# daigo0927/tf-raft

Hardware: AMD Instinct MI355X
Metric: image-pairs/sec at 448×512 iters_pred=24; final-iter EPE vs TF ref (higher is better)
Workload: dtype f32; 1 GPU; RAFT forward BASELINE configs[1]: batch 4/GPU 448x512 iters_pred=24 random weights; pairs_per_gpu=4, global_batch=4, parallelism=dp1, collective=none

## Files before the change

### tf_raft_amd/csrc/mask_upsample.hip

```cpp
#include "conv_mfma.h"

namespace {
struct MaskUpArgs {
    const float *a;
    int lda;
    const float *wp;
    const float *bias;
    const float *flow;
    float *out;
    int B, h, w;
    float scale;
};

constexpr int MU_TH = 4, MU_TW = 16, MU_LDA = 40, MU_ABUF = 64 * MU_LDA, MU_PXS = 592, MU_N = 576, MU_K = 256;

__global__ void __launch_bounds__(512) mask_upsample_kernel(MaskUpArgs p) {
    __shared__ __attribute__((aligned(16))) float sa[2 * MU_ABUF];
    __shared__ __attribute__((aligned(16))) float sm[32 * MU_PXS];
    __shared__ float2 sf[6 * 18];

    const int tid = threadIdx.x, lane = tid & 63;
    const int wv = __builtin_amdgcn_readfirstlane(tid >> 6);
    const int G = lane >> 4, LR = lane & 15;
    const int rbp = wv & 1, cg = wv >> 1;
    const int tiles_x = (p.w + MU_TW - 1) / MU_TW, tiles_y = (p.h + MU_TH - 1) / MU_TH;
    const int ntiles = p.B * tiles_x * tiles_y;
  for (int tile = blockIdx.x; tile < ntiles; tile += gridDim.x) {
    const int bid = raft_xcd_remap(tile, ntiles);
    const int tx = bid % tiles_x, ty = (bid / tiles_x) % tiles_y, b = bid / (tiles_x * tiles_y);
    const int y0 = ty * MU_TH, x0 = tx * MU_TW;
    const int M = p.B * p.h * p.w;

    const __amdgpu_buffer_rsrc_t rsa = __builtin_amdgcn_make_buffer_rsrc(
        (void *)p.a, 0, (int)((((long)M - 1) * p.lda + MU_K) * 4), 0x00020000);
    const __amdgpu_buffer_rsrc_t rsw = __builtin_amdgcn_make_buffer_rsrc((void *)p.wp, 0, MU_K * MU_N * 4, 0x00020000);

    const int spx = tid >> 3, sc4 = tid & 7;
    const int syy = y0 + (spx >> 4), sxx = x0 + (spx & 15);
    const bool sok = (syy < p.h) & (sxx < p.w);
    const unsigned soff = sok ? (unsigned)((((b * p.h + syy) * p.w + sxx) * p.lda + sc4 * 4) * 4) : RAFT_OOB;
    f32x4 ra;
    auto gload = [&](int c) { ra = __builtin_bit_cast(f32x4, __builtin_amdgcn_raw_buffer_load_b128(rsa, (int)soff, c * 128, 0)); };
    auto lstore = [&](int buf) { *(f32x4 *)(sa + buf * MU_ABUF + spx * MU_LDA + sc4 * 4) = ra; };
    const int a_lane = ((2 * rbp) * 16 + LR) * MU_LDA + G * 4;
    f32x4 fa[2][2], fb[2][9];
    auto frag_a = [&](int buf, int kk, f32x4 *f) {
#pragma unroll
        for (int i = 0; i < 2; ++i) f[i] = *(const f32x4 *)(sa + buf * MU_ABUF + a_lane + i * 16 * MU_LDA + kk * 16);
    };
    const unsigned b_lane = (unsigned)(((G * MU_N) + cg * 144 + LR) * 16);
    auto frag_b = [&](int c, int kk, f32x4 *f) {
        const unsigned row = (unsigned)((c * 8 + kk * 4) * MU_N) * 16u;
#pragma unroll
        for (int j = 0; j < 9; ++j)
            f[j] = __builtin_bit_cast(f32x4, __builtin_amdgcn_raw_buffer_load_b128(rsw, (int)(b_lane + j * 256), (int)row, 0));
    };
    f32x4 acc[2][9];
#pragma unroll
    for (int i = 0; i < 2; ++i)
#pragma unroll
        for (int j = 0; j < 9; ++j) acc[i][j] = f32x4{0.f, 0.f, 0.f, 0.f};

    constexpr int NCH = MU_K / 32;
    gload(0);
    frag_b(0, 0, fb[0]);
    if (tid < 108) {
        const int yy = y0 - 1 + tid / 18, xx = x0 - 1 + tid % 18;
        float2 f = make_float2(0.f, 0.f);
        if (yy >= 0 && yy < p.h && xx >= 0 && xx < p.w) {
            f = *(const float2 *)(p.flow + ((int64_t)(b * p.h + yy) * p.w + xx) * 2);
            f.x *= 8.f;
            f.y *= 8.f;
        }
        sf[tid] = f;
    }
    lstore(0);
    raft_barrier_lds();
    gload(1);
    frag_a(0, 0, fa[0]);
#pragma unroll
    for (int c = 0; c < NCH; ++c) {
        const int buf = c & 1;
#pragma unroll
        for (int kk = 0; kk < 2; ++kk) {
            const int cur = kk;
            if (kk == 0) {
                frag_a(buf, 1, fa[1]);
                frag_b(c, 1, fb[1]);
            } else if (c + 1 < NCH) {
                lstore(buf ^ 1);
                if (c + 2 < NCH) gload(c + 2);
                raft_barrier_lds();
                frag_a(buf ^ 1, 0, fa[0]);
                frag_b(c + 1, 0, fb[0]);
            }
#pragma unroll
            for (int r = 0; r < 4; ++r)
#pragma unroll
                for (int i = 0; i < 2; ++i)
#pragma unroll
                    for (int j = 0; j < 9; ++j)
                        acc[i][j] = __builtin_amdgcn_mfma_f32_16x16x4f32(fa[cur][i][r], fb[cur][j][r], acc[i][j], 0, 0, 0);
        }
    }

    float bias[9];
#pragma unroll
    for (int j = 0; j < 9; ++j) bias[j] = p.bias[cg * 144 + j * 16 + LR];
#pragma unroll
    for (int half = 0; half < 2; ++half) {
        raft_barrier_lds();
        if (rbp == half) {
#pragma unroll
            for (int i = 0; i < 2; ++i)
#pragma unroll
                for (int j = 0; j < 9; ++j)
#pragma unroll
                    for (int r = 0; r < 4; ++r)
                        sm[(i * 16 + 4 * G + r) * MU_PXS + cg * 144 + j * 16 + LR] = (acc[i][j][r] + bias[j]) * p.scale;
        }
        raft_barrier_lds();
#pragma unroll
        for (int t = 0; t < 4; ++t) {
            const int item = tid + 512 * t;
            const int px = item >> 6, sub = item & 63;
            const int row = 2 * half + (px >> 4), col = px & 15;
            const int y = y0 + row, x = x0 + col;
            if (y >= p.h || x >= p.w) continue;
            const float *tl = sm + px * MU_PXS + sub * 9;
            float v[9], mx = -INFINITY;
#pragma unroll
            for (int k = 0; k < 9; ++k) {
                v[k] = tl[k];
                mx = fmaxf(mx, v[k]);
            }
            float s = 0.f;
#pragma unroll
            for (int k = 0; k < 9; ++k) {
                v[k] = __builtin_amdgcn_exp2f((v[k] - mx) * 1.44269504088896341f);
                s += v[k];
            }
            const float inv = 1.0f / s;
            float ox = 0.f, oy = 0.f;
#pragma unroll
            for (int k = 0; k < 9; ++k) {
                const float2 nb = sf[(row + k / 3) * 18 + col + k % 3];
                const float wk = v[k] * inv;
                ox += wk * nb.x;
                oy += wk * nb.y;
            }
            float2 *o = (float2 *)p.out + ((int64_t)b * (8 * p.h) + (8 * y + (sub >> 3))) * (int64_t)(8 * p.w) + (8 * x + (sub & 7));
            *o = make_float2(ox, oy);
        }
// ... 20 lines not shown
```

### tf_raft_amd/csrc/conv_wino4.h

```cpp
#pragma once
#include "conv_mfma.h"

typedef float f32x2 __attribute__((ext_vector_type(2)));
typedef unsigned int u32x2 __attribute__((ext_vector_type(2)));

#include <type_traits>
#include <utility>

#ifdef RAFT_WINO4_SCALAR
struct alignas(8) w4v2 {
    float x, y;
    __device__ __forceinline__ float operator[](int i) const { return i ? y : x; }
};
__device__ __forceinline__ w4v2 operator+(w4v2 a, w4v2 b) { return {a.x + b.x, a.y + b.y}; }
__device__ __forceinline__ w4v2 operator-(w4v2 a, w4v2 b) { return {a.x - b.x, a.y - b.y}; }
__device__ __forceinline__ w4v2 operator*(float k, w4v2 a) { return {k * a.x, k * a.y}; }
#else
typedef f32x2 w4v2;
#endif

template <class F, int... I>
__device__ __forceinline__ void w4_static_for_impl(F &f, std::integer_sequence<int, I...>) {
    (f(std::integral_constant<int, I>{}), ...);
}
template <int N, class F>
__device__ __forceinline__ void w4_static_for(F &&f) {
    w4_static_for_impl(f, std::make_integer_sequence<int, N>{});
}
#define W4_TAPS(X)                                                                                                       \
    X(0) X(1) X(2) X(3) X(4) X(5) X(6) X(7) X(8) X(9) X(10) X(11) X(12) X(13) X(14) X(15) X(16) X(17) X(18) X(19) X(20) X(21)   \
    X(22) X(23) X(24) X(25) X(26) X(27) X(28) X(29) X(30) X(31) X(32) X(33) X(34) X(35)

#ifndef RAFT_WINO4_PF
#define RAFT_WINO4_PF 7
#endif
#ifdef RAFT_WINO4_NOSB
#define W4_SB()
#else
#define W4_SB() __builtin_amdgcn_sched_barrier(0)
#endif
#ifdef RAFT_WINO4_NOSNOP
#define W4_PAD ""
#else
#define W4_PAD "s_nop 1\n\t"
#endif
#define W4_MFMA4                                                                                                          \
    W4_PAD "v_mfma_f32_16x16x4_f32 %0, %2, %4, %0\n\tv_mfma_f32_16x16x4_f32 %1, %2, %6, %1\n\t"                          \
           "v_mfma_f32_16x16x4_f32 %0, %3, %5, %0\n\tv_mfma_f32_16x16x4_f32 %1, %3, %7, %1"
#ifndef RAFT_WINO4_ATAPS
#define RAFT_WINO4_ATAPS 31
#endif
#ifndef RAFT_WINO4_ABL
#define RAFT_WINO4_ABL 0
#endif

namespace wino4 {
constexpr float PA = 0.625f, PB = 1.5f;
constexpr float A2 = PA * PA, B2 = PB * PB, SS = A2 + B2, PP = A2 * B2, A3 = A2 * PA, B3 = B2 * PB;
constexpr int TW = 64, HWP = TW + 2;
constexpr int RS = 1124;
constexpr int NTHR = 256;
constexpr int PF = RAFT_WINO4_PF, NR = 8;
constexpr int W4_ATAPS = RAFT_WINO4_ATAPS;
#ifndef RAFT_WINO4_LAG
#define RAFT_WINO4_LAG 12
#endif
constexpr int LOAD_SLOT0 = 0, STORE_LAG = RAFT_WINO4_LAG;
static_assert(PF >= 1 && PF < NR, "prefetch distance must fit the fragment ring");
__device__ __forceinline__ constexpr int tap_row(int ph, int row) { return ph == 0 ? 1 + row : (ph == 1 ? 3 + row : 5 * row); }
}

#pragma clang diagnostic push
#pragma clang diagnostic ignored "-Wunused-lambda-capture"
template <int EPI, int KS = 1, int PRE = 0, int STATS = 0>
__global__ void __launch_bounds__(256, 1) conv_wino4_kernel(ConvArgs p) {
    using namespace wino4;
    static_assert(EPI == EPI_LINEAR || EPI == EPI_RELU || EPI == EPI_RES, "winograd F(4x4) kernel: linear / relu / residual epilogues");
    static_assert(KS == 1 || KS == 2, "K split: 1 or 2");
    static_assert((!PRE && !STATS) || KS == 1, "encoder variants: two row blocks per workgroup");
    constexpr int TH = KS == 1 ? 8 : 4, HH = TH + 2, HP = HH * HWP;
    constexpr int A_BUF = HH * RS + 16;
    constexpr int NA = (HP * 4 * KS + NTHR - 1) / NTHR;
    static_assert(LOAD_SLOT0 + NA - 1 + STORE_LAG < 60, "halo writes must precede the chunk's barrier (slot 60)");
    __shared__ __attribute__((aligned(16))) float smem[2 * KS * A_BUF];

    const int tid = threadIdx.x, lane = tid & 63;
    const int w = __builtin_amdgcn_readfirstlane(tid >> 6);
    const int G = lane >> 4, LR = lane & 15;
    const int rb = KS == 1 ? (w & 1) : 0, cbp = KS == 1 ? (w >> 1) : (w & 1), ks = KS == 1 ? 0 : (w >> 1);
    const int tiles_x = (p.W + TW - 1) / TW, tiles_y = (p.H + TH - 1) / TH;
    const int ntn = p.npad / 64;
    const int M = p.B * p.H * p.W;

    const int bid = raft_xcd_remap(blockIdx.x, gridDim.x);
    int mt = bid / ntn, nt = bid - mt * ntn;
#ifdef RAFT_WINO4_XCD
    {
        const int nwg = gridDim.x, xcd = blockIdx.x & 7, idx = blockIdx.x >> 3;
        if ((nwg & 7) == 0 && (ntn & 7) == 0) {
            const int per = ntn >> 3;
            nt = xcd + 8 * (idx % per);
            mt = idx / per;
        } else if ((nwg & 7) == 0 && 8 % ntn == 0) {
            const int g = 8 / ntn;
            nt = xcd % ntn;
            mt = idx * g + xcd / ntn;
        }
    }
#endif
    const int tx0 = mt % tiles_x, ty0 = (mt / tiles_x) % tiles_y, b = mt / (tiles_x * tiles_y);
    const int y0 = ty0 * TH, x0 = tx0 * TW;
    const int n0 = nt * 64;
    const int cin = p.c0 + p.c1;
    const int nch = cin >> 4;
    const int nst = nch / KS;

    const __amdgpu_buffer_rsrc_t rs0 = raft_stage_src0(p, M, p.c0), rsw = raft_stage_weights(p, 36, cin);
// ... 122 lines not shown
        }
        W[par][0][j] = (R[3][j] - SS * R[1][j]) + PP * e0;
        W[par][1][j] = (e5 - SS * R[2][j]) + PP * R[0][j];
    };
    w4v2 V[6];
    auto s2_calc = [&](const w4v2 *wr, int tx) {
        if (RAFT_WINO4_ABL & 16) {
            V[tx] = wr[tx];
            return;
        }
        if (tx == 0) {
            V[0] = (wr[4] - SS * wr[2]) + PP * wr[0];
        } else if (tx == 1) {
            const w4v2 t1 = wr[4] - B2 * wr[2], t2 = wr[3] - B2 * wr[1];
            V[1] = t1 + PA * t2;
            V[2] = t1 - PA * t2;
        } else if (tx == 3) {
            const w4v2 t1 = wr[4] - A2 * wr[2], t2 = wr[3] - A2 * wr[1];
            V[3] = t1 + PB * t2;
            V[4] = t1 - PB * t2;
        } else if (tx == 5) {
            V[5] = (wr[5] - SS * wr[3]) + PP * wr[1];
        }
    };

    next_source(0);
#pragma unroll
    for (int i = 0; i < NA; ++i) gload_item(i);
#pragma unroll
    for (int q = 0; q < PF; ++q) frag_b(q);
#pragma unroll
    for (int i = 0; i < NA; ++i) lstore_item(i, 0);
    raft_barrier_lds();
#pragma unroll
    for (int j = 0; j < 6; ++j) {
#pragma unroll
        for (int r = 0; r < 4; ++r) R[r][j] = (RAFT_WINO4_ABL & 2) ? w4v2{1.f, 1.f} : rd(0, r + 1, j, 0);
        s1_pair(0, 0, j);
    }
    s2_calc(W[0][0], 0);

    auto chunk = [&](auto buf_c, int c) {
        constexpr int BUF = decltype(buf_c)::value;
        next_source(c + 1);
        w4_static_for<6>([&](auto inst_c) {
            constexpr int inst = decltype(inst_c)::value;
            constexpr int h = inst / 3, ph = inst % 3, par = inst & 1;
            constexpr int n_h = ph == 2 ? 1 - h : h;
            constexpr int n_buf = (ph == 2 && h == 1) ? 1 - BUF : BUF;
            if (inst == 5) raft_barrier_lds();
            w4_static_for<12>([&](auto u_c) {
                constexpr int u = decltype(u_c)::value;
                constexpr int row = u / 6, tx = u % 6, j = u >> 1;
                constexpr int q = inst * 12 + u;
                constexpr int t = tap_row(ph, row) * 6 + tx;
                if (!(RAFT_WINO4_ABL & 1)) frag_b((q + PF) % 72, q + PF == 72);
                if (!(RAFT_WINO4_ABL & 2)) {
                    if constexpr (ph == 1 && (u & 1) == 0) {
                        e0 = rd(BUF, 0, j, h);
                        e5 = rd(BUF, 5, j, h);
                    }
                    if constexpr (ph == 2 && (u & 1) == 0) {
#pragma unroll
                        for (int r = 0; r < 4; ++r) R[r][j] = rd(n_buf, r + 1, j, n_h);
                    }
                }
                if constexpr ((u & 1) == 1) {
                    if constexpr (ph == 0) s1_pair(par ^ 1, 1, j);
                    if constexpr (ph == 1) s1_edge(par ^ 1, j);
                    if constexpr (ph == 2) s1_pair(par ^ 1, 0, j);
                }
                {
                    constexpr int li = q - LOAD_SLOT0, si = q - LOAD_SLOT0 - STORE_LAG;
                    if constexpr (li >= 0 && li < NA) gload_item(li);
                    if constexpr (si >= 0 && si < NA) lstore_item(si, 1 - BUF);
                }
                W4_SB();
                mma4(std::integral_constant<int, t>{}, V[tx][0], V[tx][1], fb[q & (NR - 1)]);
                W4_SB();
                if constexpr (u < 11) s2_calc(W[par][(u + 1) / 6], (u + 1) % 6);
                if constexpr (u == 11) s2_calc(W[par ^ 1][0], 0);
            });
        });
    };
    for (int st = 0; st < nst; st += 2) {
        chunk(std::integral_constant<int, 0>{}, st);
        chunk(std::integral_constant<int, 1>{}, st + 1);
    }

    asm volatile("s_nop 15\n\ts_nop 15" ::: "memory");
    __builtin_amdgcn_sched_barrier(0);

    constexpr bool HAS_E0 = EPI == EPI_RES;
    const EpiBuffers eb = raft_epi_buffers<EPI>(p, M);
    const bool interior = (y0 + TH <= p.H) & (x0 + TW <= p.W);
    int tid_e = threadIdx.x;
    asm volatile("" : "+v"(tid_e));
    const int G_e = (tid_e >> 4) & 3, LR_e = tid_e & 15, rb_e = (tid_e >> 6) & 1, cbp_e = tid_e >> 7;
    const int xb = x0 + 16 * G_e;
    const int ks_e = KS == 1 ? 0 : (tid_e >> 7), cb_e = KS == 1 ? cbp_e : ((tid_e >> 6) & 1), w_e = tid_e >> 6;
    constexpr int NROW = KS == 1 ? 4 : 2;
    unsigned bo[NROW], be[NROW];
    bool rowok[NROW];
#pragma unroll
    for (int i = 0; i < NROW; ++i) {
        const int yy = y0 + (KS == 1 ? 4 * rb_e : 2 * ks_e) + i;
        const unsigned pix0 = (unsigned)((b * p.H + yy) * p.W + xb);
        bo[i] = pix0 * p.ldo0 * 4u;
        be[i] = HAS_E0 ? pix0 * p.lde0 * 4u : 0u;
        rowok[i] = yy < p.H;
    }
    float bias2[2];
    unsigned nofs[2];
    bool nok2[2];
#pragma unroll
    for (int j = 0; j < 2; ++j) {
        const int n = n0 + (cb_e * 2 + j) * 16 + LR_e;
        nok2[j] = n < p.nvalid;
        nofs[j] = (unsigned)n * 4u;
        bias2[j] = p.bias[n];
    }
    float st1[2] = {0.f, 0.f}, st2[2] = {0.f, 0.f};
    auto emit = [&](int j, int i, int rh, const f32x2 *Y) {
        const float bias = bias2[j];
        const unsigned vo = nok2[j] ? bo[i] + nofs[j] : RAFT_OOB, ve = (HAS_E0 && nok2[j]) ? be[i] + nofs[j] : RAFT_OOB;
#pragma unroll
        for (int rr = 0; rr < 2; ++rr) {
            const int r = 2 * rh + rr;
            float xv[4] = {};
            if (HAS_E0) {
#pragma unroll
                for (int jx = 0; jx < 4; ++jx) {
                    const unsigned dead = (interior | (rowok[i] & (xb + 4 * r + jx < p.W))) ? 0u : RAFT_OOB;
                    xv[jx] = raft_buffer_load_f32(eb.e0, ve | dead, (4 * r + jx) * p.lde0 * 4);
                }
            }
#pragma unroll
            for (int jx = 0; jx < 4; ++jx) {
                const float v = raft_epi_act<EPI>(Y[jx][rr] + bias, xv[jx], 0.f, p.scale);
                if ((RAFT_WINO4_ABL & 8) && v != 12345.678f) continue;
                const unsigned dead = (interior | (rowok[i] & (xb + 4 * r + jx < p.W))) ? 0u : RAFT_OOB;
                if constexpr (STATS) {
                    unsigned dd = dead;
                    asm volatile("" : "+v"(dd));
                    const float vs = __builtin_bit_cast(float, __builtin_bit_cast(unsigned, v) & ~(unsigned)((int)dd >> 31));
                    st1[j] += vs;
                    st2[j] = fmaf(vs, vs, st2[j]);
                }
                raft_buffer_store_f32(v, eb.o0, vo | dead, (4 * r + jx) * p.ldo0 * 4);
            }
        }
    };
    f32x2 *xch = (f32x2 *)smem;
    if (KS == 2) raft_barrier_lds();
    w4_static_for<4>([&](auto jr_c) {
        constexpr int j = decltype(jr_c)::value >> 1, rh = decltype(jr_c)::value & 1;
        f32x2 T[4][6], keep[2][4];
        w4_static_for<6>([&](auto tx_c) {
            constexpr int tx = decltype(tx_c)::value;
            auto half = [&](f32x4 a) { return f32x2{a[2 * rh], a[2 * rh + 1]}; };
            const f32x2 m0 = half(acc_of(std::integral_constant<int, 2 * tx + j>{})),
                        m1 = half(acc_of(std::integral_constant<int, 2 * (6 + tx) + j>{})),
                        m2 = half(acc_of(std::integral_constant<int, 2 * (12 + tx) + j>{})),
                        m3 = half(acc_of(std::integral_constant<int, 2 * (18 + tx) + j>{})),
                        m4 = half(acc_of(std::integral_constant<int, 2 * (24 + tx) + j>{})),
                        m5 = half(acc_of(std::integral_constant<int, 2 * (30 + tx) + j>{}));
            const f32x2 sa = m1 + m2, da = m1 - m2, sb = m3 + m4, db = m3 - m4;
            T[0][tx] = m0 + (sa + sb);
            T[1][tx] = PA * da + PB * db;
            T[2][tx] = A2 * sa + B2 * sb;
            T[3][tx] = (A3 * da + B3 * db) + m5;
            __builtin_amdgcn_sched_barrier(0);
        });
#pragma unroll
        for (int i = 0; i < 4; ++i) {
            const f32x2 sa = T[i][1] + T[i][2], da = T[i][1] - T[i][2], sb = T[i][3] + T[i][4], db = T[i][3] - T[i][4];
            f32x2 Y[4];
            Y[0] = T[i][0] + (sa + sb);
            Y[1] = PA * da + PB * db;
            Y[2] = A2 * sa + B2 * sb;
            Y[3] = (A3 * da + B3 * db) + T[i][5];
            if (KS == 1) {
                emit(j, i, rh, Y);
            } else {
                const bool mine = (i >> 1) == ks_e;
#pragma unroll
                for (int jx = 0; jx < 4; ++jx) {
                    if (mine)
                        keep[i & 1][jx] = Y[jx];
                    else
                        xch[(((((j * 2 + rh) * 4 + (w_e ^ 2)) * 2 + (i & 1)) * 4 + jx) << 6) + (tid_e & 63)] = Y[jx];
                }
            }
            __builtin_amdgcn_sched_barrier(0);
        }
        if (KS == 2) {
            raft_barrier_lds();
#pragma unroll
            for (int i2 = 0; i2 < 2; ++i2) {
                f32x2 Y[4];
#pragma unroll
                for (int jx = 0; jx < 4; ++jx)
                    Y[jx] = keep[i2][jx] + xch[(((((j * 2 + rh) * 4 + w_e) * 2 + i2) * 4 + jx) << 6) + (tid_e & 63)];
                emit(j, i2, rh, Y);
            }
        }
    });
    if constexpr (STATS) {
#pragma unroll
        for (int j = 0; j < 2; ++j) {
            float s1 = st1[j], s2 = st2[j];
            s1 += __shfl_xor(s1, 16, 64);
            s2 += __shfl_xor(s2, 16, 64);
            s1 += __shfl_xor(s1, 32, 64);
            s2 += __shfl_xor(s2, 32, 64);
            const int n = n0 + (cb_e * 2 + j) * 16 + LR_e;
            if (G_e == 0) *(float2 *)(p.stats + ((long)(2 * mt + rb_e) * p.npad + n) * 2) = make_float2(s1, s2);
        }
    }
}

#pragma clang diagnostic pop
```

### tf_raft_amd/csrc/encoder.hip

```cpp
#include "conv_halo.h"
#include "conv_wino.h"

namespace {

__global__ void __launch_bounds__(256) enc_prep_kernel(const float *__restrict__ img, const float *__restrict__ img_b,
                                                       int64_t npix_a, f32x4 *__restrict__ out, int64_t npix, int affine) {
    const int64_t i = (int64_t)blockIdx.x * 256 + threadIdx.x;
    if (i >= npix) return;
    const float *src = i < npix_a ? img + 3 * i : img_b + 3 * (i - npix_a);
    float r = src[0], g = src[1], b = src[2];
    if (affine) {
#pragma clang fp contract(off)
        r = 2.f * (r / 255.f) - 1.f;
        g = 2.f * (g / 255.f) - 1.f;
        b = 2.f * (b / 255.f) - 1.f;
    }
    out[i] = f32x4{r, g, b, 0.f};
}

__global__ void __launch_bounds__(1024) in_finalize_kernel(const float *__restrict__ part, int tiles, int npad, int C,
                                                           const float *__restrict__ gamma, const float *__restrict__ beta,
                                                           double inv_count, float *__restrict__ scale,
                                                           float *__restrict__ shift) {
    __shared__ double sh[2][16][64];
// ... 19 lines not shown
        a = (a + a1) + (a2 + a3);
        q = (q + q1) + (q2 + q3);
    }
    sh[0][grp][threadIdx.x & 63] = a;
    sh[1][grp][threadIdx.x & 63] = q;
    __syncthreads();
    if (grp == 0 && c < C) {
        for (int g = 1; g < 16; ++g) {
            a += sh[0][g][threadIdx.x];
            q += sh[1][g][threadIdx.x];
        }
        const double mean = a * inv_count;
        double var = q * inv_count - mean * mean;
        if (var < 0.0) var = 0.0;
        const double sc = (double)gamma[c] / sqrt(var + 1e-3);
        scale[(int64_t)img * C + c] = (float)sc;
        shift[(int64_t)img * C + c] = (float)((double)beta[c] - mean * sc);
    }
}

__global__ void __launch_bounds__(256) res_merge_kernel(const f32x4 *__restrict__ x, const float *__restrict__ xs,
                                                        const float *__restrict__ xh, const f32x4 *__restrict__ f,
                                                        const float *__restrict__ fs, const float *__restrict__ fh,
                                                        f32x4 *__restrict__ y, int64_t total4, int c4n, int64_t pix_per_img,
                                                        int mode) {
    const int64_t i = (int64_t)blockIdx.x * 256 + threadIdx.x;
    if (i >= total4) return;
    const int c4 = (int)(i % c4n);
    const int64_t img = (i / c4n) / pix_per_img;
    const f32x4 s = *(const f32x4 *)(fs + (img * c4n + c4) * 4), h = *(const f32x4 *)(fh + (img * c4n + c4) * 4);
    f32x4 v = f[i];
#pragma unroll
    for (int e = 0; e < 4; ++e) v[e] = fmaxf(fmaf(v[e], s[e], h[e]), 0.f);
    if (mode == 0) {
        f32x4 xv = x[i];
        if (xs) {
            const f32x4 s2 = *(const f32x4 *)(xs + (img * c4n + c4) * 4), h2 = *(const f32x4 *)(xh + (img * c4n + c4) * 4);
#pragma unroll
            for (int e = 0; e < 4; ++e) xv[e] = fmaf(xv[e], s2[e], h2[e]);
        }
#pragma unroll
        for (int e = 0; e < 4; ++e) v[e] = fmaxf(xv[e] + v[e], 0.f);
    }
    y[i] = v;
}

enum EncKind { ENC_3x3_S1, ENC_3x3_S2, ENC_1x1_S2, ENC_1x1_S1, ENC_STEM };

template <int KH, int KW, int EPI, int STRIDE, int PRE, int STATS, int STEM>
int launch_tile(const ConvArgs &a, int th, int tn, hipStream_t s) {
    return raft_launch_conv_halo_tile<KH, KW, EPI, STRIDE, PRE, STATS, STEM, false>(a, th, tn, s);
}

int enc_conv(const ConvArgs &a, EncKind kind, int epi, int th, int tn, hipStream_t s) {
    const bool pre = a.pre_scale != nullptr, stats = a.stats != nullptr;
    switch (kind) {
        case ENC_3x3_S1:
            if (epi == EPI_LINEAR && stats && !pre) return launch_tile<3, 3, EPI_LINEAR, 1, 0, 1, 0>(a, th, tn, s);
            if (epi == EPI_LINEAR && stats && pre) return launch_tile<3, 3, EPI_LINEAR, 1, 1, 1, 0>(a, th, tn, s);
            if (epi == EPI_RELU && !pre) return launch_tile<3, 3, EPI_RELU, 1, 0, 0, 0>(a, th, tn, s);
            if (epi == EPI_RES && !pre) return launch_tile<3, 3, EPI_RES, 1, 0, 0, 0>(a, th, tn, s);
            break;
        case ENC_3x3_S2:
            if (epi == EPI_LINEAR && stats && !pre) return launch_tile<3, 3, EPI_LINEAR, 2, 0, 1, 0>(a, th, tn, s);
            if (epi == EPI_RELU && !pre) return launch_tile<3, 3, EPI_RELU, 2, 0, 0, 0>(a, th, tn, s);
            break;
        case ENC_1x1_S2:
            if (epi == EPI_LINEAR && stats && !pre) return launch_tile<1, 1, EPI_LINEAR, 2, 0, 1, 0>(a, th, tn, s);
            if (epi == EPI_LINEAR && !stats && !pre) return launch_tile<1, 1, EPI_LINEAR, 2, 0, 0, 0>(a, th, tn, s);
            break;
        case ENC_1x1_S1:
            if (epi == EPI_LINEAR && !stats && !pre) return launch_tile<1, 1, EPI_LINEAR, 1, 0, 0, 0>(a, th, tn, s);
// ... 120 lines not shown
        a.e0 = res; a.lde0 = cout;
        a.pre_scale = pre_sc; a.pre_shift = pre_sh;
        a.stats = (inorm && slot >= 0) ? b.part : nullptr;
        int th, tn;
        enc_pick(Ho, cw.npad, &th, &tn);
        const bool plain = pre_sc == nullptr && a.stats == nullptr;
        int rc = wino4  ? raft_launch_conv_wino4(a, epi, s, raft_wino4_plan(n, Ho, Wo, a.c0, a.c1, a.npad, plain, hint))
                 : wino ? raft_launch_conv_wino(a, epi, s, raft_wino_plan(n, Ho, Wo, a.c0, a.c1, a.npad, plain, hint))
                        : enc_conv(a, kind, epi, th, tn, s);
        if (rc != RAFT_OK) return rc;
        if (a.stats) {
            const int tiles = wino4  ? 2 * ((Ho + 7) / 8) * ((Wo + 63) / 64)
                              : wino ? 2 * ((Ho + 3) / 4) * ((Wo + 31) / 32)
                                     : ((Ho + th - 1) / th) * ((Wo + 15) / 16);
            dim3 grid((cout + 63) / 64, n);
            in_finalize_kernel<<<grid, 1024, 0, s>>>(b.part, tiles, cw.npad, cout, gamma, beta, 1.0 / ((double)Ho * Wo),
                                                     ss_slot[slot][0], ss_slot[slot][1]);
            rc = raft_launch_status();
        }
        return rc;
    };
    auto merge = [&](const float *x, const float *xs, const float *xh, const float *f, const float *fs, const float *fh,
                     float *y, int Ho, int Wo, int C, int mode) -> int {
        const int64_t total4 = (int64_t)n * Ho * Wo * C / 4;
        res_merge_kernel<<<raft_ceil_div(total4, 256), 256, 0, s>>>((const f32x4 *)x, xs, xh, (const f32x4 *)f, fs, fh,
                                                                    (f32x4 *)y, total4, C / 4, (int64_t)Ho * Wo, mode);
        return raft_launch_status();
    };

    int Hc, Wc, pt, pl;
    same_pad(H, 7, 2, &Hc, &pt);
    same_pad(W, 7, 2, &Wc, &pl);
    int C = w->c0;
    if (inorm) {
        RAFT_TRY(conv(ENC_STEM, w->conv1, b.img4, 0, H, W, Hc, Wc, pt, pl, C, EPI_LINEAR, b.r1, nullptr, nullptr, nullptr,
                          0, w->in_gamma[0], w->in_beta[0]));
        RAFT_TRY(merge(nullptr, nullptr, nullptr, b.r1, ss_slot[0][0], ss_slot[0][1], b.x, Hc, Wc, C, 1));
    } else {
        RAFT_TRY(conv(ENC_STEM, w->conv1, b.img4, 0, H, W, Hc, Wc, pt, pl, C, EPI_RELU, b.x, nullptr, nullptr, nullptr,
                          -1, nullptr, nullptr));
    }

    float *x = b.x, *y = b.y;
    const int widths[3] = {w->c1, w->c2, w->c3};
    for (int blk = 0; blk < 6; ++blk) {
        const int F = widths[blk / 2];
        const int stride = (blk == 2 || blk == 4) ? 2 : 1;
        const raft_conv_weights &c1 = w->block[blk][0], &c2 = w->block[blk][1], &cd = w->block[blk][2];
        int Ho = Hc, Wo = Wc, p1t = 1, p1l = 1;
        if (stride == 2) {
            same_pad(Hc, 3, 2, &Ho, &p1t);
            same_pad(Wc, 3, 2, &Wo, &p1l);
        }
        const EncKind k1 = stride == 2 ? ENC_3x3_S2 : ENC_3x3_S1;
        const int ni = 1 + blk * 3;
        const bool w4 = raft_enc_stage_wino4(blk / 2, n, Ho, Wo, F, hint);
        const raft_conv_weights *w44a = w4 ? &w->block_w44[blk][0] : nullptr, *w44b = w4 ? &w->block_w44[blk][1] : nullptr;
        if (inorm) {
            RAFT_TRY(conv(k1, c1, x, C, Hc, Wc, Ho, Wo, p1t, p1l, F, EPI_LINEAR, b.r1, nullptr, nullptr, nullptr, 0,
                              w->in_gamma[ni], w->in_beta[ni], &w->block_w[blk][0], w44a));
            RAFT_TRY(conv(ENC_3x3_S1, c2, b.r1, F, Ho, Wo, Ho, Wo, 1, 1, F, EPI_LINEAR, b.r2, nullptr, ss_slot[0][0],
                              ss_slot[0][1], 1, w->in_gamma[ni + 1], w->in_beta[ni + 1], &w->block_w[blk][1], w44b));
            if (stride == 2) {
                RAFT_REQUIRE(cd.wp != nullptr, RAFT_E_NULL);
                RAFT_TRY(conv(ENC_1x1_S2, cd, x, C, Hc, Wc, Ho, Wo, 0, 0, F, EPI_LINEAR, b.rd, nullptr, nullptr, nullptr, 2,
                                  w->in_gamma[ni + 2], w->in_beta[ni + 2]));
                RAFT_TRY(merge(b.rd, ss_slot[2][0], ss_slot[2][1], b.r2, ss_slot[1][0], ss_slot[1][1], y, Ho, Wo, F, 0));
            } else {
                RAFT_TRY(merge(x, nullptr, nullptr, b.r2, ss_slot[1][0], ss_slot[1][1], y, Ho, Wo, F, 0));
            }
        } else {
            RAFT_TRY(conv(k1, c1, x, C, Hc, Wc, Ho, Wo, p1t, p1l, F, EPI_RELU, b.r1, nullptr, nullptr, nullptr, -1, nullptr,
                              nullptr, &w->block_w[blk][0], w44a));
            const float *shortcut = x;
            if (stride == 2) {
                RAFT_REQUIRE(cd.wp != nullptr, RAFT_E_NULL);
                RAFT_TRY(conv(ENC_1x1_S2, cd, x, C, Hc, Wc, Ho, Wo, 0, 0, F, EPI_LINEAR, b.rd, nullptr, nullptr, nullptr, -1,
                                  nullptr, nullptr));
                shortcut = b.rd;
            }
            RAFT_TRY(conv(ENC_3x3_S1, c2, b.r1, F, Ho, Wo, Ho, Wo, 1, 1, F, EPI_RES, y, shortcut, nullptr, nullptr, -1,
                              nullptr, nullptr, &w->block_w[blk][1], w44b));
        }
        float *t = x; x = y; y = t;
        C = F; Hc = Ho; Wc = Wo;
    }
    return conv(ENC_1x1_S1, w->conv2, x, C, Hc, Wc, Hc, Wc, 0, 0, w->cout, EPI_LINEAR, out, nullptr, nullptr, nullptr, -1,
                nullptr, nullptr);
}
```

### tf_raft_amd/csrc/host_util.hip

```cpp
#include <stddef.h>
#include <stdint.h>
#include <stdio.h>
#include <stdlib.h>
#include <string.h>

#include <atomic>
#include <mutex>

#include "common.h"

namespace {
struct Crc32cTable {
    uint32_t t[8][256];
    Crc32cTable() {
        for (uint32_t i = 0; i < 256; ++i) {
            uint32_t c = i;
            for (int k = 0; k < 8; ++k) c = (c >> 1) ^ (0x82f63b78u & (0u - (c & 1u)));
            t[0][i] = c;
        }
        for (uint32_t i = 0; i < 256; ++i)
            for (int s = 1; s < 8; ++s) t[s][i] = (t[s - 1][i] >> 8) ^ t[0][t[s - 1][i] & 0xffu];
    }
};
}

extern "C" uint32_t raft_crc32c(uint32_t crc, const void *data, size_t n) {
    static const Crc32cTable tab;
    const unsigned char *p = (const unsigned char *)data;
    uint32_t c = ~crc;
    while (n && ((uintptr_t)p & 7u)) {
        c = (c >> 8) ^ tab.t[0][(c ^ *p++) & 0xffu];
        --n;
    }
    while (n >= 8) {
        uint64_t w;
        __builtin_memcpy(&w, p, 8);
        w ^= c;
        c = tab.t[7][w & 0xff] ^ tab.t[6][(w >> 8) & 0xff] ^ tab.t[5][(w >> 16) & 0xff] ^ tab.t[4][(w >> 24) & 0xff] ^
            tab.t[3][(w >> 32) & 0xff] ^ tab.t[2][(w >> 40) & 0xff] ^ tab.t[1][(w >> 48) & 0xff] ^ tab.t[0][w >> 56];
        p += 8;
        n -= 8;
    }
    while (n--) c = (c >> 8) ^ tab.t[0][(c ^ *p++) & 0xffu];
    return ~c;
}

namespace {
const char *const kOptNames[RAFT_OPT_COUNT] = {
    "RAFT_CONV_WINO", "RAFT_SMALL_WINO", "RAFT_GRU_WINO", "RAFT_GRU_WINO4", "RAFT_WINO_TNW", "RAFT_WINO_SB",
    "RAFT_WINO_CK", "RAFT_WINO1D_TM",
    "RAFT_LOOKUP_FUSED", "RAFT_ONDEMAND_BLOCK", "RAFT_ENC_WINO",
    "RAFT_WINO_KS", "RAFT_CONV_WINO4", "RAFT_WINO4_KS", "RAFT_MASK_FUSED", "RAFT_ENC_WINO4", "RAFT_CONVC2_KS", "RAFT_CONVF2_KS",
    "RAFT_EVENT_FENCE", "RAFT_CORR_XCD", "RAFT_CORR_POOL",
};
constexpr int kTileEntries = 16;
struct TileRule {
    int npad, taps, code;
};
struct Options {
    std::atomic<int> val[RAFT_OPT_COUNT];
    std::atomic<bool> set[RAFT_OPT_COUNT];
    int env_val[RAFT_OPT_COUNT];
    bool env_set[RAFT_OPT_COUNT];
    std::mutex tile_mu;
    char tile_text[256], tile_env[256];
    TileRule tile_rules[kTileEntries];
    int n_tile_rules, tile_all;
    Options() {
        for (int i = 0; i < RAFT_OPT_COUNT; ++i) {
            const char *e = getenv(kOptNames[i]);
            env_set[i] = e && *e;
            env_val[i] = env_set[i] ? atoi(e) : 0;
            val[i].store(env_val[i]);
            set[i].store(env_set[i]);
        }
        const char *e = getenv("RAFT_CONV_TILE");
        snprintf(tile_env, sizeof(tile_env), "%s", e ? e : "");
        parse_tiles(tile_env);
    }
    void parse_tiles(const char *text) {
        snprintf(tile_text, sizeof(tile_text), "%s", text ? text : "");
        n_tile_rules = 0;
        tile_all = -1;
        if (!tile_text[0]) return;
        if (!strchr(tile_text, ':')) {
            tile_all = atoi(tile_text);
// ... 92 lines not shown
```

### tf_raft_amd/csrc/launch_plan.h

```cpp
#pragma once

#include <stdint.h>

#include "../../include/raft_hip.h"

enum RaftOptionId {
    RAFT_OPT_CONV_WINO, RAFT_OPT_SMALL_WINO, RAFT_OPT_GRU_WINO, RAFT_OPT_GRU_WINO4, RAFT_OPT_WINO_TNW, RAFT_OPT_WINO_SB,
    RAFT_OPT_WINO_CK, RAFT_OPT_WINO1D_TM,
    RAFT_OPT_LOOKUP_FUSED, RAFT_OPT_ONDEMAND_BLOCK, RAFT_OPT_ENC_WINO,
    RAFT_OPT_WINO_KS, RAFT_OPT_CONV_WINO4, RAFT_OPT_WINO4_KS, RAFT_OPT_MASK_FUSED, RAFT_OPT_ENC_WINO4, RAFT_OPT_CONVC2_KS, RAFT_OPT_CONVF2_KS,
    RAFT_OPT_EVENT_FENCE, RAFT_OPT_CORR_XCD, RAFT_OPT_CORR_POOL,
    RAFT_OPT_COUNT
};
int raft_opt(int id, int dflt);
bool raft_opt_is_set(int id);
int raft_opt_conv_tile(int npad, int taps, bool (*valid)(int code, int npad));

#ifdef __HIP__
#define RAFT_HOST_DEVICE __host__ __device__
#else
#define RAFT_HOST_DEVICE
#endif
RAFT_HOST_DEVICE static inline int raft_xcd_remap(int bid, int nwg) {
    const int xcd = bid & 7, q = nwg >> 3, r = nwg & 7;
    return (xcd < r ? xcd * (q + 1) : r * (q + 1) + (xcd - r) * q) + (bid >> 3);
}

enum RaftConvFamily { RAFT_FAM_HALO, RAFT_FAM_WINO, RAFT_FAM_WINO1D, RAFT_FAM_WINO4 };
struct HaloPlan { int th, tn; };
struct WinoPlan { int tnw, sb, ck, ks; };
struct Wino1dPlan { int mo, tnw, tm, ck; };
struct Wino4Plan { int ks; };
struct ConvChoice { int family; HaloPlan halo; WinoPlan wino; Wino1dPlan wino1d; Wino4Plan wino4; const raft_conv_weights *wt; };
typedef const raft_conv_weights *RaftWeights;
static inline ConvChoice raft_choice(HaloPlan p, RaftWeights wt = nullptr) { ConvChoice c = {RAFT_FAM_HALO}; c.halo = p; c.wt = wt; return c; }
static inline ConvChoice raft_choice(WinoPlan p, RaftWeights wt = nullptr) { ConvChoice c = {RAFT_FAM_WINO}; c.wino = p; c.wt = wt; return c; }
static inline ConvChoice raft_choice(Wino1dPlan p, RaftWeights wt = nullptr) { ConvChoice c = {RAFT_FAM_WINO1D}; c.wino1d = p; c.wt = wt; return c; }
static inline ConvChoice raft_choice(Wino4Plan p, RaftWeights wt = nullptr) { ConvChoice c = {RAFT_FAM_WINO4}; c.wino4 = p; c.wt = wt; return c; }

static inline bool raft_halo_code_valid(int code, int npad) {
    const int th = (code - 100) / 10, tn = (code - 100) % 10;
    return code >= 100 && (th == 4 || th == 7 || th == 8) && (tn == 1 || tn == 2) && npad % (64 * tn) == 0;
}

// ... 122 lines not shown
            p.gru[l] = raft_choice(raft_halo_plan(B, h, w, gw[l][0]->npad, kh, kw, hint), gw[l][0]);
    }
    return p;
}

static inline ConvChoice raft_gru_ctx_plan(const raft_basic_update_weights &wt, int pass, int B, int h, int w, int hint) {
    const raft_conv_weights &w4 = pass == 0 ? wt.gru_ctx1_w4 : wt.gru_ctx2_w4;
    const int kh = pass == 0 ? 1 : 5;
    if (w4.wp != nullptr && (raft_opt(RAFT_OPT_GRU_WINO4, RAFT_GRU_WINO4_DEFAULT) & (pass == 0 ? 1 : 4)))
        return raft_choice(raft_wino1d_plan(B, h, w, 128, 0, w4.npad, kh, 4, hint), &w4);
    const raft_conv_weights &wc = pass == 0 ? wt.gru_ctx1 : wt.gru_ctx2;
    return raft_choice(raft_halo_plan(B, h, w, wc.npad, kh, 6 - kh, hint), &wc);
}

struct SmallLoopPlan { ConvChoice convc1, convf2, conv, gru_zr, gru_q, fh1; };

static inline SmallLoopPlan raft_small_loop_plan(const raft_small_update_weights &wt, int B, int h, int w, int hint) {
    SmallLoopPlan p = {};
    const int mask = raft_opt(RAFT_OPT_SMALL_WINO, RAFT_SMALL_WINO_DEFAULT);
    auto conv3x3 = [&](int bit, const raft_conv_weights &direct, const raft_conv_weights &w2, int c0, int c1) {
        return (mask & bit) && w2.wp != nullptr ? raft_choice(raft_wino_plan(B, h, w, c0, c1, w2.npad, true, hint), &w2)
                                                : raft_choice(raft_halo_plan(B, h, w, direct.npad, 3, 3, hint), &direct);
    };
    p.convc1 = raft_choice(raft_halo_plan(B, h, w, wt.convc1.npad, 1, 1, hint), &wt.convc1);
    p.convf2 = raft_choice(raft_halo_plan(B, h, w, wt.convf2.npad, 3, 3, hint), &wt.convf2);
    p.conv = conv3x3(1, wt.conv, wt.conv_w, 128, 0);
    p.gru_zr = conv3x3(2, wt.gru_zr, wt.gru_zr_w, 96, 160);
    p.gru_q = conv3x3(4, wt.gru_q, wt.gru_q_w, 96, 160);
    p.fh1 = conv3x3(8, wt.fh1, wt.fh1_w, 96, 0);
    return p;
}

static inline bool raft_enc_wino() { return raft_opt(RAFT_OPT_ENC_WINO, 1) != 0; }
static inline bool raft_enc_stage_wino4(int stage, int n, int Ho, int Wo, int F, int hint) {
    const int mask = raft_enc_wino() ? raft_opt(RAFT_OPT_ENC_WINO4, 7) : 0;
    return ((mask >> stage) & 1) &&
           (raft_opt_is_set(RAFT_OPT_ENC_WINO4) || (int64_t)n * ((Ho + 7) / 8) * ((Wo + 63) / 64) * ((F + 63) / 64) * hint > 256);
}
```

Before: 387.1 image-pairs/s.

## Interleave weight loads with MFMAs and split epilogue rows across both wave halves

```diff
diff --git a/tf_raft_amd/csrc/mask_upsample.hip b/tf_raft_amd/csrc/mask_upsample.hip
--- a/tf_raft_amd/csrc/mask_upsample.hip
+++ b/tf_raft_amd/csrc/mask_upsample.hip
@@ -14,10 +14,12 @@
 
 constexpr int MU_TH = 4, MU_TW = 16, MU_LDA = 40, MU_ABUF = 64 * MU_LDA, MU_PXS = 592, MU_N = 576, MU_K = 256;
 
+typedef float f32x2 __attribute__((ext_vector_type(2)));
+
 __global__ void __launch_bounds__(512) mask_upsample_kernel(MaskUpArgs p) {
     __shared__ __attribute__((aligned(16))) float sa[2 * MU_ABUF];
     __shared__ __attribute__((aligned(16))) float sm[32 * MU_PXS];
-    __shared__ float2 sf[6 * 18];
+    __shared__ float2 sf[512];
 
     const int tid = threadIdx.x, lane = tid & 63;
     const int wv = __builtin_amdgcn_readfirstlane(tid >> 6);
@@ -25,15 +27,15 @@
     const int rbp = wv & 1, cg = wv >> 1;
     const int tiles_x = (p.w + MU_TW - 1) / MU_TW, tiles_y = (p.h + MU_TH - 1) / MU_TH;
     const int ntiles = p.B * tiles_x * tiles_y;
+    const int M = p.B * p.h * p.w;
+    const __amdgpu_buffer_rsrc_t rsa = __builtin_amdgcn_make_buffer_rsrc(
+        (void *)p.a, 0, (int)((((long)M - 1) * p.lda + MU_K) * 4), 0x00020000);
+    const __amdgpu_buffer_rsrc_t rsw = __builtin_amdgcn_make_buffer_rsrc((void *)p.wp, 0, MU_K * MU_N * 4, 0x00020000);
+    const __amdgpu_buffer_rsrc_t rsf = __builtin_amdgcn_make_buffer_rsrc((void *)p.flow, 0, M * 8, 0x00020000);
   for (int tile = blockIdx.x; tile < ntiles; tile += gridDim.x) {
     const int bid = raft_xcd_remap(tile, ntiles);
     const int tx = bid % tiles_x, ty = (bid / tiles_x) % tiles_y, b = bid / (tiles_x * tiles_y);
     const int y0 = ty * MU_TH, x0 = tx * MU_TW;
-    const int M = p.B * p.h * p.w;
-
-    const __amdgpu_buffer_rsrc_t rsa = __builtin_amdgcn_make_buffer_rsrc(
-        (void *)p.a, 0, (int)((((long)M - 1) * p.lda + MU_K) * 4), 0x00020000);
-    const __amdgpu_buffer_rsrc_t rsw = __builtin_amdgcn_make_buffer_rsrc((void *)p.wp, 0, MU_K * MU_N * 4, 0x00020000);
 
     const int spx = tid >> 3, sc4 = tid & 7;
     const int syy = y0 + (spx >> 4), sxx = x0 + (spx & 15);
@@ -42,18 +44,16 @@
     f32x4 ra;
     auto gload = [&](int c) { ra = __builtin_bit_cast(f32x4, __builtin_amdgcn_raw_buffer_load_b128(rsa, (int)soff, c * 128, 0)); };
     auto lstore = [&](int buf) { *(f32x4 *)(sa + buf * MU_ABUF + spx * MU_LDA + sc4 * 4) = ra; };
-    const int a_lane = ((2 * rbp) * 16 + LR) * MU_LDA + G * 4;
+    const int a_lane = (rbp * 16 + LR) * MU_LDA + G * 4;
     f32x4 fa[2][2], fb[2][9];
     auto frag_a = [&](int buf, int kk, f32x4 *f) {
 #pragma unroll
-        for (int i = 0; i < 2; ++i) f[i] = *(const f32x4 *)(sa + buf * MU_ABUF + a_lane + i * 16 * MU_LDA + kk * 16);
+        for (int i = 0; i < 2; ++i) f[i] = *(const f32x4 *)(sa + buf * MU_ABUF + a_lane + i * 32 * MU_LDA + kk * 16);
     };
     const unsigned b_lane = (unsigned)(((G * MU_N) + cg * 144 + LR) * 16);
-    auto frag_b = [&](int c, int kk, f32x4 *f) {
+    auto frag_b = [&](int c, int kk, int j) {
         const unsigned row = (unsigned)((c * 8 + kk * 4) * MU_N) * 16u;
-#pragma unroll
-        for (int j = 0; j < 9; ++j)
-            f[j] = __builtin_bit_cast(f32x4, __builtin_amdgcn_raw_buffer_load_b128(rsw, (int)(b_lane + j * 256), (int)row, 0));
+        return __builtin_bit_cast(f32x4, __builtin_amdgcn_raw_buffer_load_b128(rsw, (int)(b_lane + j * 256), (int)row, 0));
     };
     f32x4 acc[2][9];
 #pragma unroll
@@ -61,64 +61,62 @@
 #pragma unroll
         for (int j = 0; j < 9; ++j) acc[i][j] = f32x4{0.f, 0.f, 0.f, 0.f};
 
-    constexpr int NCH = MU_K / 32;
+    const int fy = y0 - 1 + tid / 18, fx = x0 - 1 + tid % 18;
+    const bool fok = (tid < 108) & (fy >= 0) & (fy < p.h) & (fx >= 0) & (fx < p.w);
+    const unsigned foff = fok ? (unsigned)(((b * p.h + fy) * p.w + fx) * 8) : RAFT_OOB;
     gload(0);
-    frag_b(0, 0, fb[0]);
-    if (tid < 108) {
-        const int yy = y0 - 1 + tid / 18, xx = x0 - 1 + tid % 18;
-        float2 f = make_float2(0.f, 0.f);
-        if (yy >= 0 && yy < p.h && xx >= 0 && xx < p.w) {
-            f = *(const float2 *)(p.flow + ((int64_t)(b * p.h + yy) * p.w + xx) * 2);
-            f.x *= 8.f;
-            f.y *= 8.f;
-        }
-        sf[tid] = f;
-    }
+    const f32x2 rf = __builtin_bit_cast(f32x2, __builtin_amdgcn_raw_buffer_load_b64(rsf, (int)foff, 0, 0));
+#pragma unroll
+    for (int j = 0; j < 9; ++j) fb[0][j] = frag_b(0, 0, j);
     lstore(0);
+    sf[tid] = make_float2(rf.x * 8.f, rf.y * 8.f);
     raft_barrier_lds();
     gload(1);
     frag_a(0, 0, fa[0]);
+
+    constexpr int NCH = MU_K / 32;
+    float bias[9];
 #pragma unroll
     for (int c = 0; c < NCH; ++c) {
         const int buf = c & 1;
 #pragma unroll
         for (int kk = 0; kk < 2; ++kk) {
-            const int cur = kk;
+            const bool more = kk == 0 || c + 1 < NCH;
+            const int nc = kk == 0 ? c : c + 1;
             if (kk == 0) {
                 frag_a(buf, 1, fa[1]);
-                frag_b(c, 1, fb[1]);
             } else if (c + 1 < NCH) {
                 lstore(buf ^ 1);
                 if (c + 2 < NCH) gload(c + 2);
                 raft_barrier_lds();
                 frag_a(buf ^ 1, 0, fa[0]);
-                frag_b(c + 1, 0, fb[0]);
+            } else {
+#pragma unroll
+                for (int j = 0; j < 9; ++j) bias[j] = p.bias[cg * 144 + j * 16 + LR];
             }
+            __builtin_amdgcn_sched_barrier(0);
 #pragma unroll
             for (int r = 0; r < 4; ++r)
 #pragma unroll
                 for (int i = 0; i < 2; ++i)
 #pragma unroll
-                    for (int j = 0; j < 9; ++j)
-                        acc[i][j] = __builtin_amdgcn_mfma_f32_16x16x4f32(fa[cur][i][r], fb[cur][j][r], acc[i][j], 0, 0, 0);
+                    for (int j = 0; j < 9; ++j) {
+                        const bool slot = more && r == 0 && i == 0;
+                        if (slot) fb[kk ^ 1][j] = frag_b(nc, kk ^ 1, j);
+                        acc[i][j] = __builtin_amdgcn_mfma_f32_16x16x4f32(fa[kk][i][r], fb[kk][j][r], acc[i][j], 0, 0, 0);
+                        if (slot) __builtin_amdgcn_sched_barrier(0);
+                    }
         }
     }
 
-    float bias[9];
-#pragma unroll
-    for (int j = 0; j < 9; ++j) bias[j] = p.bias[cg * 144 + j * 16 + LR];
 #pragma unroll
     for (int half = 0; half < 2; ++half) {
-        raft_barrier_lds();
-        if (rbp == half) {
+        if (half == 1) raft_barrier_lds();
 #pragma unroll
-            for (int i = 0; i < 2; ++i)
+        for (int j = 0; j < 9; ++j)
 #pragma unroll
-                for (int j = 0; j < 9; ++j)
-#pragma unroll
-                    for (int r = 0; r < 4; ++r)
-                        sm[(i * 16 + 4 * G + r) * MU_PXS + cg * 144 + j * 16 + LR] = (acc[i][j][r] + bias[j]) * p.scale;
-        }
+            for (int r = 0; r < 4; ++r)
+                sm[(rbp * 16 + 4 * G + r) * MU_PXS + cg * 144 + j * 16 + LR] = (acc[half][j][r] + bias[j]) * p.scale;
         raft_barrier_lds();
 #pragma unroll
         for (int t = 0; t < 4; ++t) {
```

Result: no change. 389.1 image-pairs/s, median of 6 (+0.5%).

## Fuse encoder stem norm into first block and prefetch residuals in wino4 epilogue

Applied to the files above, without the earlier changes.

```diff
diff --git a/tf_raft_amd/csrc/conv_wino4.h b/tf_raft_amd/csrc/conv_wino4.h
--- a/tf_raft_amd/csrc/conv_wino4.h
+++ b/tf_raft_amd/csrc/conv_wino4.h
@@ -50,8 +50,34 @@
 #ifndef RAFT_WINO4_ATAPS
 #define RAFT_WINO4_ATAPS 31
 #endif
+#ifndef RAFT_WINO4_RES_AHEAD
+#define RAFT_WINO4_RES_AHEAD 3
+#endif
 #ifndef RAFT_WINO4_ABL
 #define RAFT_WINO4_ABL 0
+#endif
+
+#ifdef RAFT_WINO4_STAMP
+__device__ unsigned long long *raft_wino4_stamps;
+template <bool REAL = false>
+__device__ __forceinline__ void w4_stamp(int slot) {
+    unsigned long long t;
+    __builtin_amdgcn_sched_barrier(0);
+    if (REAL)
+        asm volatile("s_memrealtime %0\n\ts_waitcnt lgkmcnt(0)" : "=s"(t)::"memory");
+    else
+        asm volatile("s_memtime %0\n\ts_waitcnt lgkmcnt(0)" : "=s"(t)::"memory");
+    __builtin_amdgcn_sched_barrier(0);
+    const __amdgpu_buffer_rsrc_t rs = raft_stage_rsrc(raft_wino4_stamps, (int)(gridDim.x * 128u));
+    const unsigned off = (threadIdx.x == 0 && slot < 16) ? blockIdx.x * 128u + (unsigned)slot * 8u : RAFT_OOB;
+    __builtin_amdgcn_raw_buffer_store_b32((unsigned)t, rs, (int)off, 0, 0);
+    __builtin_amdgcn_raw_buffer_store_b32((unsigned)(t >> 32), rs, (int)off, 4, 0);
+}
+#define W4_STAMP(slot) w4_stamp(slot)
+#define W4_STAMP_REAL(slot) w4_stamp<true>(slot)
+#else
+#define W4_STAMP(slot)
+#define W4_STAMP_REAL(slot)
 #endif
 
 namespace wino4 {
@@ -83,6 +109,8 @@
     constexpr int NA = (HP * 4 * KS + NTHR - 1) / NTHR;
     static_assert(LOAD_SLOT0 + NA - 1 + STORE_LAG < 60, "halo writes must precede the chunk's barrier (slot 60)");
     __shared__ __attribute__((aligned(16))) float smem[2 * KS * A_BUF];
+    W4_STAMP_REAL(13);
+    W4_STAMP(0);
 
     const int tid = threadIdx.x, lane = tid & 63;
     const int w = __builtin_amdgcn_readfirstlane(tid >> 6);
@@ -271,6 +299,7 @@
 #pragma unroll
     for (int i = 0; i < NA; ++i) lstore_item(i, 0);
     raft_barrier_lds();
+    W4_STAMP(1);
 #pragma unroll
     for (int j = 0; j < 6; ++j) {
 #pragma unroll
@@ -281,6 +310,7 @@
 
     auto chunk = [&](auto buf_c, int c) {
         constexpr int BUF = decltype(buf_c)::value;
+        W4_STAMP(c < 8 ? 2 + c : 16);
         next_source(c + 1);
         w4_static_for<6>([&](auto inst_c) {
             constexpr int inst = decltype(inst_c)::value;
@@ -326,6 +356,7 @@
         chunk(std::integral_constant<int, 0>{}, st);
         chunk(std::integral_constant<int, 1>{}, st + 1);
     }
+    W4_STAMP(10);
 
     asm volatile("s_nop 15\n\ts_nop 15" ::: "memory");
     __builtin_amdgcn_sched_barrier(0);
@@ -360,20 +391,34 @@
         bias2[j] = p.bias[n];
     }
     float st1[2] = {0.f, 0.f}, st2[2] = {0.f, 0.f};
+    constexpr int RES_AHEAD = KS == 2 ? 1 : (RAFT_WINO4_RES_AHEAD < NROW ? RAFT_WINO4_RES_AHEAD : NROW);
+    float xres[RES_AHEAD][2][4] = {};
+    auto load_res = [&](int s) {
+        if constexpr (HAS_E0) {
+            if (s >= 4 * NROW) return;
+            const int j = (s / NROW) >> 1, rh = (s / NROW) & 1, i = s % NROW;
+            const unsigned ve = nok2[j] ? be[i] + nofs[j] : RAFT_OOB;
+            int xb_l = xb;
+            asm volatile("" : "+v"(xb_l));
+#pragma unroll
+            for (int rr = 0; rr < 2; ++rr) {
+                const int r = 2 * rh + rr;
+#pragma unroll
+                for (int jx = 0; jx < 4; ++jx) {
+                    const unsigned dead = (interior | (rowok[i] & (xb_l + 4 * r + jx < p.W))) ? 0u : RAFT_OOB;
+                    xres[s % RES_AHEAD][rr][jx] = raft_buffer_load_f32(eb.e0, ve | dead, (4 * r + jx) * p.lde0 * 4);
+                }
+            }
+            __builtin_amdgcn_sched_barrier(0);
+        }
+    };
     auto emit = [&](int j, int i, int rh, const f32x2 *Y) {
         const float bias = bias2[j];
-        const unsigned vo = nok2[j] ? bo[i] + nofs[j] : RAFT_OOB, ve = (HAS_E0 && nok2[j]) ? be[i] + nofs[j] : RAFT_OOB;
+        const unsigned vo = nok2[j] ? bo[i] + nofs[j] : RAFT_OOB;
 #pragma unroll
         for (int rr = 0; rr < 2; ++rr) {
             const int r = 2 * rh + rr;
-            float xv[4] = {};
-            if (HAS_E0) {
-#pragma unroll
-                for (int jx = 0; jx < 4; ++jx) {
-                    const unsigned dead = (interior | (rowok[i] & (xb + 4 * r + jx < p.W))) ? 0u : RAFT_OOB;
-                    xv[jx] = raft_buffer_load_f32(eb.e0, ve | dead, (4 * r + jx) * p.lde0 * 4);
-                }
-            }
+            const float *xv = xres[((2 * j + rh) * NROW + i) % RES_AHEAD][rr];
 #pragma unroll
             for (int jx = 0; jx < 4; ++jx) {
                 const float v = raft_epi_act<EPI>(Y[jx][rr] + bias, xv[jx], 0.f, p.scale);
@@ -392,8 +437,10 @@
     };
     f32x2 *xch = (f32x2 *)smem;
     if (KS == 2) raft_barrier_lds();
+#pragma unroll
+    for (int s = 0; s < RES_AHEAD; ++s) load_res(s);
     w4_static_for<4>([&](auto jr_c) {
-        constexpr int j = decltype(jr_c)::value >> 1, rh = decltype(jr_c)::value & 1;
+        constexpr int jr = decltype(jr_c)::value, j = jr >> 1, rh = jr & 1;
         f32x2 T[4][6], keep[2][4];
         w4_static_for<6>([&](auto tx_c) {
             constexpr int tx = decltype(tx_c)::value;
@@ -421,6 +468,7 @@
             Y[3] = (A3 * da + B3 * db) + T[i][5];
             if (KS == 1) {
                 emit(j, i, rh, Y);
+                load_res(jr * NROW + i + RES_AHEAD);
             } else {
                 const bool mine = (i >> 1) == ks_e;
 #pragma unroll
@@ -442,6 +490,7 @@
                 for (int jx = 0; jx < 4; ++jx)
                     Y[jx] = keep[i2][jx] + xch[(((((j * 2 + rh) * 4 + w_e) * 2 + i2) * 4 + jx) << 6) + (tid_e & 63)];
                 emit(j, i2, rh, Y);
+                load_res(jr * NROW + i2 + RES_AHEAD);
             }
         }
     });
@@ -457,6 +506,12 @@
             if (G_e == 0) *(float2 *)(p.stats + ((long)(2 * mt + rb_e) * p.npad + n) * 2) = make_float2(s1, s2);
         }
     }
+    W4_STAMP(11);
+#ifdef RAFT_WINO4_STAMP
+    asm volatile("s_waitcnt vmcnt(0)" ::: "memory");
+#endif
+    W4_STAMP(12);
+    W4_STAMP_REAL(14);
 }
 
 #pragma clang diagnostic pop
diff --git a/tf_raft_amd/csrc/encoder.hip b/tf_raft_amd/csrc/encoder.hip
--- a/tf_raft_amd/csrc/encoder.hip
+++ b/tf_raft_amd/csrc/encoder.hip
@@ -75,12 +75,16 @@
     f32x4 v = f[i];
 #pragma unroll
     for (int e = 0; e < 4; ++e) v[e] = fmaxf(fmaf(v[e], s[e], h[e]), 0.f);
-    if (mode == 0) {
+    if (mode != 1) {
         f32x4 xv = x[i];
         if (xs) {
             const f32x4 s2 = *(const f32x4 *)(xs + (img * c4n + c4) * 4), h2 = *(const f32x4 *)(xh + (img * c4n + c4) * 4);
 #pragma unroll
             for (int e = 0; e < 4; ++e) xv[e] = fmaf(xv[e], s2[e], h2[e]);
+            if (mode == 2) {
+#pragma unroll
+                for (int e = 0; e < 4; ++e) xv[e] = fmaxf(xv[e], 0.f);
+            }
         }
 #pragma unroll
         for (int e = 0; e < 4; ++e) v[e] = fmaxf(xv[e] + v[e], 0.f);
@@ -267,7 +271,11 @@
     same_pad(H, 7, 2, &Hc, &pt);
     same_pad(W, 7, 2, &Wc, &pl);
     int C = w->c0;
-    if (inorm) {
+    const bool stem_fused = inorm && raft_enc_stem_fused();
+    if (stem_fused) {
+        RAFT_TRY(conv(ENC_STEM, w->conv1, b.img4, 0, H, W, Hc, Wc, pt, pl, C, EPI_LINEAR, b.rd, nullptr, nullptr, nullptr,
+                          2, w->in_gamma[0], w->in_beta[0]));
+    } else if (inorm) {
         RAFT_TRY(conv(ENC_STEM, w->conv1, b.img4, 0, H, W, Hc, Wc, pt, pl, C, EPI_LINEAR, b.r1, nullptr, nullptr, nullptr,
                           0, w->in_gamma[0], w->in_beta[0]));
         RAFT_TRY(merge(nullptr, nullptr, nullptr, b.r1, ss_slot[0][0], ss_slot[0][1], b.x, Hc, Wc, C, 1));
@@ -292,8 +300,10 @@
         const bool w4 = raft_enc_stage_wino4(blk / 2, n, Ho, Wo, F, hint);
         const raft_conv_weights *w44a = w4 ? &w->block_w44[blk][0] : nullptr, *w44b = w4 ? &w->block_w44[blk][1] : nullptr;
         if (inorm) {
-            RAFT_TRY(conv(k1, c1, x, C, Hc, Wc, Ho, Wo, p1t, p1l, F, EPI_LINEAR, b.r1, nullptr, nullptr, nullptr, 0,
-                              w->in_gamma[ni], w->in_beta[ni], &w->block_w[blk][0], w44a));
+            const bool raw_in = stem_fused && blk == 0;
+            RAFT_TRY(conv(k1, c1, raw_in ? b.rd : x, C, Hc, Wc, Ho, Wo, p1t, p1l, F, EPI_LINEAR, b.r1, nullptr,
+                              raw_in ? ss_slot[2][0] : nullptr, raw_in ? ss_slot[2][1] : nullptr, 0, w->in_gamma[ni], w->in_beta[ni],
+                              &w->block_w[blk][0], w44a));
             RAFT_TRY(conv(ENC_3x3_S1, c2, b.r1, F, Ho, Wo, Ho, Wo, 1, 1, F, EPI_LINEAR, b.r2, nullptr, ss_slot[0][0],
                               ss_slot[0][1], 1, w->in_gamma[ni + 1], w->in_beta[ni + 1], &w->block_w[blk][1], w44b));
             if (stride == 2) {
@@ -301,6 +311,8 @@
                 RAFT_TRY(conv(ENC_1x1_S2, cd, x, C, Hc, Wc, Ho, Wo, 0, 0, F, EPI_LINEAR, b.rd, nullptr, nullptr, nullptr, 2,
                                   w->in_gamma[ni + 2], w->in_beta[ni + 2]));
                 RAFT_TRY(merge(b.rd, ss_slot[2][0], ss_slot[2][1], b.r2, ss_slot[1][0], ss_slot[1][1], y, Ho, Wo, F, 0));
+            } else if (raw_in) {
+                RAFT_TRY(merge(b.rd, ss_slot[2][0], ss_slot[2][1], b.r2, ss_slot[1][0], ss_slot[1][1], y, Ho, Wo, F, 2));
             } else {
                 RAFT_TRY(merge(x, nullptr, nullptr, b.r2, ss_slot[1][0], ss_slot[1][1], y, Ho, Wo, F, 0));
             }
diff --git a/tf_raft_amd/csrc/host_util.hip b/tf_raft_amd/csrc/host_util.hip
--- a/tf_raft_amd/csrc/host_util.hip
+++ b/tf_raft_amd/csrc/host_util.hip
@@ -51,7 +51,7 @@
     "RAFT_WINO_CK", "RAFT_WINO1D_TM",
     "RAFT_LOOKUP_FUSED", "RAFT_ONDEMAND_BLOCK", "RAFT_ENC_WINO",
     "RAFT_WINO_KS", "RAFT_CONV_WINO4", "RAFT_WINO4_KS", "RAFT_MASK_FUSED", "RAFT_ENC_WINO4", "RAFT_CONVC2_KS", "RAFT_CONVF2_KS",
-    "RAFT_EVENT_FENCE", "RAFT_CORR_XCD", "RAFT_CORR_POOL",
+    "RAFT_EVENT_FENCE", "RAFT_CORR_XCD", "RAFT_CORR_POOL", "RAFT_ENC_STEM_FUSED",
 };
 constexpr int kTileEntries = 16;
 struct TileRule {
diff --git a/tf_raft_amd/csrc/launch_plan.h b/tf_raft_amd/csrc/launch_plan.h
--- a/tf_raft_amd/csrc/launch_plan.h
+++ b/tf_raft_amd/csrc/launch_plan.h
@@ -9,7 +9,7 @@
     RAFT_OPT_WINO_CK, RAFT_OPT_WINO1D_TM,
     RAFT_OPT_LOOKUP_FUSED, RAFT_OPT_ONDEMAND_BLOCK, RAFT_OPT_ENC_WINO,
     RAFT_OPT_WINO_KS, RAFT_OPT_CONV_WINO4, RAFT_OPT_WINO4_KS, RAFT_OPT_MASK_FUSED, RAFT_OPT_ENC_WINO4, RAFT_OPT_CONVC2_KS, RAFT_OPT_CONVF2_KS,
-    RAFT_OPT_EVENT_FENCE, RAFT_OPT_CORR_XCD, RAFT_OPT_CORR_POOL,
+    RAFT_OPT_EVENT_FENCE, RAFT_OPT_CORR_XCD, RAFT_OPT_CORR_POOL, RAFT_OPT_ENC_STEM_FUSED,
     RAFT_OPT_COUNT
 };
 int raft_opt(int id, int dflt);
@@ -198,6 +198,7 @@
 }
 
 static inline bool raft_enc_wino() { return raft_opt(RAFT_OPT_ENC_WINO, 1) != 0; }
+static inline bool raft_enc_stem_fused() { return raft_opt(RAFT_OPT_ENC_STEM_FUSED, 1) != 0; }
 static inline bool raft_enc_stage_wino4(int stage, int n, int Ho, int Wo, int F, int hint) {
     const int mask = raft_enc_wino() ? raft_opt(RAFT_OPT_ENC_WINO4, 7) : 0;
     return ((mask >> stage) & 1) &&
```

Result: no change. 388.4 image-pairs/s before, 390.3 image-pairs/s after (median of 6 runs) (+0.5%).
